# robflynnyh/dynamic-asr-eval

Measured on AMD Instinct MI355X. Metric: audio-sec/s dynamic-eval (fwd+1 adapt step), higher is better.
Workload: dtype f32; 1 GPU; run_dynamic_eval_full: 1 h Earnings-22-shape recording per step (360000 frames, seq_len 16384, overlap 14336, offline, MADGRAD lr 9e-05, 6 freq masks <=34), SCConformerXL 6x768 V+1=4096 seeded weights; windows_per_recording=169, chains_per_gpu=2, lockstep_group=4, hip_graphs=True, pcie_inclusive=False

## Files before the change

### dynamic-asr-eval_amd/csrc/ctc.hip

```cpp
#include "common.h"
#include "libm_f32.h"

namespace {

namespace glm = dyn::glm;

constexpr int SCAN_T = 1024;
template <int ITEMS> struct ScanCfg { static constexpr int PD = ITEMS >= 8 ? 2 : ITEMS >= 4 ? 4 : 8; };

__device__ __forceinline__ bool better(float v, int i, float bv, int bi) { return v > bv || (v == bv && i < bi); }

__global__ __launch_bounds__(256) void argmax_rows_kernel(const float* __restrict__ x, int32_t* __restrict__ ids,
                                                           int64_t rows, int C, int64_t ld, float* __restrict__ vals) {
    const int lane = threadIdx.x & 63, w = threadIdx.x >> 6;
    for (int64_t row = (int64_t)blockIdx.x * 4 + w; row < rows; row += (int64_t)gridDim.x * 4) {
        const float* xr = x + row * ld;
        float bv = -INFINITY;
        int bi = 0x7fffffff;
        for (int c = lane; c < C; c += 64) {
            const float v = xr[c];
            if (better(v, c, bv, bi)) { bv = v; bi = c; }
        }
#pragma unroll
        for (int o = 32; o > 0; o >>= 1) {
            const float ov = __shfl_xor(bv, o, 64);
            const int oi = __shfl_xor(bi, o, 64);
            if (better(ov, oi, bv, bi)) { bv = ov; bi = oi; }
        }
        if (lane == 0) {
            ids[row] = bi == 0x7fffffff ? 0 : bi;
            if (vals) vals[row] = bv;
        }
    }
}

__global__ __launch_bounds__(1024) void ctc_collapse_kernel(const int32_t* __restrict__ ids, int32_t* __restrict__ out,
                                                             int32_t* __restrict__ out_len, int64_t T, int64_t stride,
                                                             int blank) {
    __shared__ int wsum[16];
    __shared__ int base;
    const int64_t b = blockIdx.x;
    const int32_t* in = ids + b * stride;
    int32_t* o = out + b * stride;
    const int lane = threadIdx.x & 63, w = threadIdx.x >> 6;
    if (threadIdx.x == 0) base = 0;
    __syncthreads();
    for (int64_t t0 = 0; t0 < T; t0 += 1024) {
        const int64_t t = t0 + threadIdx.x;
        int id = -1, keep = 0;
        if (t < T) {
            id = in[t];
            const int prev = t > 0 ? in[t - 1] : -1;
            keep = (id != blank && id != prev) ? 1 : 0;
        }
        int incl = keep;
#pragma unroll
        for (int o2 = 1; o2 < 64; o2 <<= 1) {
            const int n = __shfl_up(incl, o2, 64);
            if (lane >= o2) incl += n;
        }
        if (lane == 63) wsum[w] = incl;
        __syncthreads();
        int woff = 0;
        for (int k = 0; k < w; ++k) woff += wsum[k];
        const int b0 = base;
        if (keep) o[b0 + woff + incl - 1] = id;
        __syncthreads();
        if (threadIdx.x == 1023) base = b0 + woff + incl;
        __syncthreads();
    }
    if (threadIdx.x == 0) out_len[b] = base;
}


struct CtcDims {
    int64_t T_max, B, C;
    int64_t lp_st, lp_sb;
    int64_t S_max;
    int64_t L_max;
    int blank;
};

__global__ __launch_bounds__(1024) void ctc_prep_kernel(const int32_t* __restrict__ targets, const int32_t* __restrict__ tlen,
                                                        int32_t* __restrict__ prev_same, int32_t* __restrict__ is_last,
                                                        int64_t S_max) {
    extern __shared__ int32_t tg_s[];
    const int64_t b = blockIdx.x;
    const int S = tlen[b];
    const int32_t* tg = targets + b * S_max;
    for (int k = threadIdx.x; k < S; k += blockDim.x) tg_s[k] = tg[k];
    __syncthreads();
    const int lane = threadIdx.x & 63, w = threadIdx.x >> 6, nw = blockDim.x >> 6;
    for (int k = w; k < S; k += nw) {
        const int c = tg_s[k];
        int pv = -1;
        for (int j0 = k - 1; j0 >= 0; j0 -= 64) {
            const int j = j0 - lane;
            const unsigned long long hit = __ballot(j >= 0 && tg_s[j] == c);
            if (hit) { pv = j0 - (__ffsll((long long)hit) - 1); break; }
        }
        int last = 1;
        for (int j0 = k + 1; j0 < S; j0 += 64) {
            const int j = j0 + lane;
            if (__ballot(j < S && tg_s[j] == c)) { last = 0; break; }
        }
        if (lane == 0) {
            prev_same[b * S_max + k] = pv;
            is_last[b * S_max + k] = last;
        }
    }
}

__global__ __launch_bounds__(256) void ctc_gather_kernel(const float* __restrict__ lp, const int32_t* __restrict__ targets,
                                                          const int32_t* __restrict__ ilen, const int32_t* __restrict__ tlen,
                                                          float* __restrict__ slab, CtcDims d) {
    const int64_t t = blockIdx.x, b = blockIdx.y;
    if (t >= ilen[b]) return;
    const int L = 2 * tlen[b] + 1;
    const float* row = lp + t * d.lp_st + b * d.lp_sb;
    const int32_t* tg = targets + b * d.S_max;
    float* out = slab + (b * d.T_max + t) * d.L_max;
    for (int s = threadIdx.x; s < L; s += blockDim.x) out[s] = row[(s & 1) ? tg[s >> 1] : d.blank];
}

__device__ __forceinline__ float lse3(float a, float b, float c, const double* tab) {
    float m = fmaxf(a, fmaxf(b, c));
    if (m == -INFINITY) m = 0.f;
    const float e = __fadd_rn(__fadd_rn(glm::exp_nonpos(__fsub_rn(a, m), tab), glm::exp_nonpos(__fsub_rn(b, m), tab)), glm::exp_nonpos(__fsub_rn(c, m), tab));
    return __fadd_rn(glm::logf_(e, tab), m);
}

template <int ITEMS>
__device__ __forceinline__ void ctc_alpha_body(float* rows, const double* tab, const float* __restrict__ slab, const int32_t* __restrict__ targets,
                                               const int32_t* __restrict__ ilen, const int32_t* __restrict__ tlen,
                                               float* __restrict__ alpha, float* __restrict__ nll, const CtcDims& d) {
    const int SCAN_T = blockDim.x;
    const int64_t b = blockIdx.x;
    const int T = ilen[b], S = tlen[b], L = 2 * S + 1;
    const int32_t* tg = targets + b * d.S_max;
    const float* sl = slab + b * d.T_max * d.L_max;
    float* al = alpha + b * d.T_max * d.L_max;
    float* prev = rows;
    float* cur = rows + d.L_max;
    constexpr int PD = ScanCfg<ITEMS>::PD;
    bool skip[ITEMS];
    float ring[ITEMS][PD];
#pragma unroll
    for (int j = 0; j < ITEMS; ++j) {
        const int s = threadIdx.x + j * SCAN_T;
        skip[j] = (s < L) && (s & 1) && s >= 3 && tg[s >> 1] != tg[(s >> 1) - 1];
        float v = -INFINITY;
        if (s < L && T > 0) {
            if (s == 0) v = sl[0];
            else if (s == 1) v = sl[1];
            al[s] = v;
            prev[s] = v;
        }
#pragma unroll
        for (int u = 0; u < PD; ++u) ring[j][u] = (s < L && 1 + u < T) ? sl[(int64_t)(1 + u) * d.L_max + s] : 0.f;
    }
    __syncthreads();
    for (int t0 = 1; t0 < T; t0 += PD) {
#pragma unroll
        for (int u = 0; u < PD; ++u) {
            const int t = t0 + u;
            if (t < T) {
#pragma unroll
                for (int j = 0; j < ITEMS; ++j) {
                    const int s = threadIdx.x + j * SCAN_T;
                    const float lpv = ring[j][u];
                    const int tn = t + PD;
                    ring[j][u] = (s < L && tn < T) ? sl[(int64_t)tn * d.L_max + s] : 0.f;
                    if (s < L) {
                        const float a = prev[s];
                        const float bb = s >= 1 ? prev[s - 1] : -INFINITY;
                        const float c = skip[j] ? prev[s - 2] : -INFINITY;
                        const float v = __fadd_rn(lse3(a, bb, c, tab), lpv);
                        cur[s] = v;
                        al[(int64_t)t * d.L_max + s] = v;
                    }
                }
                __syncthreads();
                float* tmp = prev; prev = cur; cur = tmp;
            }
        }
    }
    if (threadIdx.x == 0) {
        float r = INFINITY;
        if (T > 0) {
            const float l1 = prev[L - 1];
            if (S == 0) r = -l1;
            else {
                const float l2 = prev[L - 2];
                float m = fmaxf(l1, l2);
                if (m == -INFINITY) m = 0.f;
                r = -__fadd_rn(glm::logf_(__fadd_rn(glm::exp_nonpos(__fsub_rn(l1, m), tab), glm::exp_nonpos(__fsub_rn(l2, m), tab)), tab), m);
            }
        }
        nll[b] = r;
    }
}

template <int ITEMS>
__device__ __forceinline__ void ctc_beta_body(float* rows, const double* tab, const float* __restrict__ slab, const int32_t* __restrict__ targets,
                                              const int32_t* __restrict__ ilen, const int32_t* __restrict__ tlen,
                                              float* __restrict__ alpha, const CtcDims& d) {
    const int SCAN_T = blockDim.x;
    const int64_t b = blockIdx.x;
    const int T = ilen[b], S = tlen[b], L = 2 * S + 1;
    if (T <= 0) return;
    const int32_t* tg = targets + b * d.S_max;
    const float* sl = slab + b * d.T_max * d.L_max;
    float* al = alpha + b * d.T_max * d.L_max;
    float* prev = rows;
    float* cur = rows + d.L_max;
    constexpr int PD = ScanCfg<ITEMS>::PD;
    bool skip[ITEMS];
    float ring[ITEMS][PD];
#pragma unroll
    for (int j = 0; j < ITEMS; ++j) {
        const int s = threadIdx.x + j * SCAN_T;
        skip[j] = (s + 2 < L) && (s & 1) && tg[s >> 1] != tg[(s >> 1) + 1];
        if (s < L) {
            float v = -INFINITY;
            if (s == L - 1 || s == L - 2) v = sl[(int64_t)(T - 1) * d.L_max + s];
            prev[s] = v;
            al[(int64_t)(T - 1) * d.L_max + s] = v;
        }
#pragma unroll
        for (int u = 0; u < PD; ++u) {
            const int t = T - 2 - u;
            ring[j][u] = (s < L && t >= 0) ? sl[(int64_t)t * d.L_max + s] : 0.f;
        }
    }
    __syncthreads();
    for (int t0 = T - 2; t0 >= 0; t0 -= PD) {
#pragma unroll
        for (int u = 0; u < PD; ++u) {
            const int t = t0 - u;
            if (t >= 0) {
#pragma unroll
                for (int j = 0; j < ITEMS; ++j) {
                    const int s = threadIdx.x + j * SCAN_T;
                    const float lpv = ring[j][u];
                    const int tn = t - PD;
                    ring[j][u] = (s < L && tn >= 0) ? sl[(int64_t)tn * d.L_max + s] : 0.f;
                    if (s < L) {
                        const float a = prev[s];
                        const float bb = s + 1 < L ? prev[s + 1] : -INFINITY;
                        const float c = skip[j] ? prev[s + 2] : -INFINITY;
                        const float v = __fadd_rn(lse3(a, bb, c, tab), lpv);
                        cur[s] = v;
                        al[(int64_t)t * d.L_max + s] = v;
                    }
                }
                __syncthreads();
                float* tmp = prev; prev = cur; cur = tmp;
            }
        }
    }
}

template <int ITEMS>
__global__ __launch_bounds__(1024) void ctc_scan_kernel(const float* __restrict__ slab, const int32_t* __restrict__ targets,
                                                         const int32_t* __restrict__ ilen, const int32_t* __restrict__ tlen,
                                                         float* __restrict__ alpha, float* __restrict__ beta, float* __restrict__ nll,
                                                         CtcDims d) {
    extern __shared__ __attribute__((aligned(16))) double scan_lds[];
    glm::stage_table(scan_lds);
    float* rows = (float*)(scan_lds + glm::TABLE_DOUBLES);
    if (blockIdx.y == 0) ctc_alpha_body<ITEMS>(rows, scan_lds, slab, targets, ilen, tlen, alpha, nll, d);
    else ctc_beta_body<ITEMS>(rows, scan_lds, slab, targets, ilen, tlen, beta, d);
}

__device__ __forceinline__ float log_add_pair(float lcab, float ab, const double* tab) {
    if (lcab == -INFINITY) return ab;
    const float mx = lcab < ab ? ab : lcab;
    return __fadd_rn(glm::logf_(__fadd_rn(glm::exp_nonpos(__fsub_rn(lcab, mx), tab), glm::exp_nonpos(__fsub_rn(ab, mx), tab)), tab), mx);
}

__global__ __launch_bounds__(256) void ctc_grad_kernel(const float* __restrict__ lp, const float* __restrict__ alpha_,
                                                        const float* __restrict__ beta_,
                                                        const int32_t* __restrict__ targets, const int32_t* __restrict__ prev_same,
                                                        const int32_t* __restrict__ is_last, const int32_t* __restrict__ ilen, const int32_t* __restrict__ tlen,
                                                        const float* __restrict__ nll, float* __restrict__ grad, int64_t g_st,
                                                        int64_t g_sb, float grad_scale, int mean_reduction, CtcDims d) {
    extern __shared__ __attribute__((aligned(16))) double grad_lds[];
    const int64_t t = blockIdx.x, b = blockIdx.y;
    const int T = ilen[b], S = tlen[b], L = 2 * S + 1;
    float* gr = grad + t * g_st + b * g_sb;
    if (t >= T) {
        for (int c = threadIdx.x; c < d.C; c += blockDim.x) gr[c] = 0.f;
        return;
    }
    const double* tab = grad_lds;
    float* ab = (float*)(grad_lds + glm::TABLE_DOUBLES);
    glm::stage_table(grad_lds);
    float g = grad_scale;
    if (mean_reduction) g = (grad_scale / (float)d.B) / (float)(S > 0 ? S : 1);
    const float* row = lp + t * d.lp_st + b * d.lp_sb;
    const float* ar = alpha_ + (b * d.T_max + t) * d.L_max;
    const float* br = beta_ + (b * d.T_max + t) * d.L_max;
    const int32_t* tg = targets + b * d.S_max;
    const int32_t* pv = prev_same + b * d.S_max;
    const float nl = nll[b];
    for (int s = threadIdx.x; s < L; s += blockDim.x) ab[s] = __fadd_rn(ar[s], br[s]);
    __syncthreads();
    for (int c = threadIdx.x; c < d.C; c += blockDim.x) gr[c] = __fmul_rn(glm::expf_(row[c], tab), g);
    __syncthreads();
    if (threadIdx.x == 0) {
        float lcab = -INFINITY;
        for (int k = S; k >= 0; --k) lcab = log_add_pair(lcab, ab[2 * k], tab);
        const float lpb = row[d.blank];
        gr[d.blank] = __fmul_rn(__fsub_rn(glm::expf_(lpb, tab), glm::expf_(__fsub_rn(__fadd_rn(lcab, nl), lpb), tab)), g);
    }
    for (int k = (int)threadIdx.x - 64; k < S; k += (int)blockDim.x - 64) {
        if (k < 0 || !is_last[b * d.S_max + k]) continue;
        const int c = tg[k];
        float lcab = -INFINITY;
        for (int j = k; j >= 0; j = pv[j]) lcab = log_add_pair(lcab, ab[2 * j + 1], tab);
        const float lpc = row[c];
        gr[c] = __fmul_rn(__fsub_rn(glm::expf_(lpc, tab), glm::expf_(__fsub_rn(__fadd_rn(lcab, nl), lpc), tab)), g);
    }
}

__global__ void ctc_loss_reduce_kernel(const float* __restrict__ nll, const int32_t* __restrict__ tlen, float* loss, int64_t B,
                                       int mean_reduction) {
    if (threadIdx.x != 0 || blockIdx.x != 0) return;
    float s = 0.f;
    for (int64_t b = 0; b < B; ++b) {
        const int S = tlen[b];
        s += mean_reduction ? nll[b] / (float)(S > 0 ? S : 1) : nll[b];
    }
    *loss = mean_reduction ? s / (float)B : s;
}

inline int64_t align_up(int64_t v, int64_t a) { return (v + a - 1) / a * a; }

struct CtcWs {
    float* slab; float* alpha; float* beta; float* nll; int32_t* prev_same; int32_t* is_last;
    int64_t total;
};

CtcWs carve(void* ws, int64_t T, int64_t B, int64_t S_max) {
    const int64_t L = 2 * S_max + 1;
    CtcWs w;
    char* p = (char*)ws;
    int64_t off = 0;
    w.slab = (float*)(p + off); off += align_up(B * T * L * 4, 256);
    w.alpha = (float*)(p + off); off += align_up(B * T * L * 4, 256);
    w.beta = (float*)(p + off); off += align_up(B * T * L * 4, 256);
    w.nll = (float*)(p + off); off += align_up(B * 4, 256);
    w.prev_same = (int32_t*)(p + off); off += align_up((B * S_max + 1) * 4, 256);
    w.is_last = (int32_t*)(p + off); off += align_up((B * S_max + 1) * 4, 256);
    w.total = off;
    return w;
}

}

extern "C" int dyn_ctc_greedy(const float* log_probs, int64_t B, int64_t T, int64_t C, int64_t ld, int32_t blank,
                              int32_t* argmax_ids, int32_t* out_ids, int32_t* out_len, void* stream) {
    DYN_REQUIRE(log_probs && argmax_ids && out_ids && out_len && B >= 0 && T >= 0 && C > 0 && ld >= C, DYN_E_ARG,
                "dyn_ctc_greedy: bad arguments");
    if (B == 0) return DYN_OK;
    hipStream_t st = (hipStream_t)stream;
    if (T > 0) {
        int64_t g = dyn::cdiv(B * T, 4);
        if (g > 8192) g = 8192;
        hipLaunchKernelGGL(argmax_rows_kernel, dim3((unsigned)g), dim3(256), 0, st, log_probs, argmax_ids, B * T, (int)C, ld, (float*)nullptr);
    }
    hipLaunchKernelGGL(ctc_collapse_kernel, dim3((unsigned)B), dim3(1024), 0, st, argmax_ids, out_ids, out_len, T, T, (int)blank);
    return dyn::check_launch("dyn_ctc_greedy");
}

extern "C" int dyn_argmax_rows(const float* x, int64_t rows, int64_t C, int64_t ld, int32_t* ids, float* vals, void* stream) {
    DYN_REQUIRE(x && ids && rows >= 0 && C > 0 && ld >= C, DYN_E_ARG, "dyn_argmax_rows: bad arguments");
    if (rows == 0) return DYN_OK;
    int64_t g = dyn::cdiv(rows, 4);
    if (g > 8192) g = 8192;
    hipLaunchKernelGGL(argmax_rows_kernel, dim3((unsigned)g), dim3(256), 0, (hipStream_t)stream, x, ids, rows, (int)C, ld, vals);
    return dyn::check_launch("dyn_argmax_rows");
}

extern "C" int64_t dyn_ctc_loss_workspace_bytes(int64_t T, int64_t B, int64_t S_max) {
    return carve(nullptr, T, B, S_max > 0 ? S_max : 1).total;
}

extern "C" int dyn_ctc_loss_workspace_layout(int64_t T, int64_t B, int64_t S_max, int64_t* offsets4, int64_t* row_len) {
    DYN_REQUIRE(offsets4 && row_len && T > 0 && B > 0 && S_max >= 0, DYN_E_ARG, "dyn_ctc_loss_workspace_layout: bad arguments");
    const int64_t Sm = S_max > 0 ? S_max : 1;
    const CtcWs w = carve(nullptr, T, B, Sm);
    offsets4[0] = (char*)w.slab - (char*)nullptr;
    offsets4[1] = (char*)w.alpha - (char*)nullptr;
    offsets4[2] = (char*)w.beta - (char*)nullptr;
    offsets4[3] = (char*)w.nll - (char*)nullptr;
    *row_len = 2 * Sm + 1;
    return DYN_OK;
}

namespace {
__global__ __launch_bounds__(256) void libm_f32_kernel(const float* __restrict__ x, int64_t n, float* y_exp, float* y_log, float* y_np) {
    __shared__ double tab[glm::TABLE_DOUBLES];
    glm::stage_table(tab);
    __syncthreads();
    for (int64_t i = (int64_t)blockIdx.x * blockDim.x + threadIdx.x; i < n; i += (int64_t)gridDim.x * blockDim.x) {
        const float v = x[i];
        if (y_exp) y_exp[i] = glm::expf_(v, tab);
        if (y_log) y_log[i] = glm::logf_(v, tab);
        if (y_np) y_np[i] = glm::exp_nonpos(v, tab);
    }
}
}

extern "C" int dyn_libm_f32(const float* x, int64_t n, float* y_exp, float* y_log, float* y_exp_nonpos, void* stream) {
    DYN_REQUIRE(x && n >= 0, DYN_E_ARG, "dyn_libm_f32: bad arguments");
    if (n == 0) return DYN_OK;
    int64_t g = dyn::cdiv(n, 256);
    if (g > 4096) g = 4096;
    hipLaunchKernelGGL(libm_f32_kernel, dim3((unsigned)g), dim3(256), 0, (hipStream_t)stream, x, n, y_exp, y_log, y_exp_nonpos);
    return dyn::check_launch("dyn_libm_f32");
}

extern "C" int dyn_ctc_loss(const float* log_probs, int64_t T, int64_t B, int64_t C, int64_t lp_stride_t, int64_t lp_stride_b,
                            const int32_t* targets, int64_t S_max, const int32_t* input_lengths, const int32_t* target_lengths,
                            int32_t blank, int32_t reduction, float grad_scale, float* loss, float* nll_per_sample,
                            float* grad, int64_t g_stride_t, int64_t g_stride_b, void* workspace, int64_t workspace_bytes,
                            void* stream) {
    DYN_REQUIRE(log_probs && targets && input_lengths && target_lengths && loss && T > 0 && B > 0 && C > 0 && S_max >= 0 &&
                    blank >= 0 && blank < C && (reduction == 0 || reduction == 1),
                DYN_E_ARG, "dyn_ctc_loss: bad arguments");
    const int64_t Sm = S_max > 0 ? S_max : 1;
    const int64_t L = 2 * Sm + 1;
    DYN_REQUIRE(L <= 8 * SCAN_T, DYN_E_UNSUPPORTED, "dyn_ctc_loss: lattice width %lld > %d unsupported", (long long)L, 8 * SCAN_T);
    CtcWs w = carve(workspace, T, B, Sm);
    DYN_REQUIRE(workspace && workspace_bytes >= w.total, DYN_E_WORKSPACE, "dyn_ctc_loss: workspace %lld < %lld bytes",
                (long long)workspace_bytes, (long long)w.total);
    CtcDims d;
    d.T_max = T; d.B = B; d.C = C; d.lp_st = lp_stride_t; d.lp_sb = lp_stride_b; d.S_max = Sm; d.L_max = L; d.blank = blank;
    hipStream_t st = (hipStream_t)stream;
    hipLaunchKernelGGL(ctc_prep_kernel, dim3((unsigned)B), dim3(1024), (size_t)Sm * sizeof(int32_t), st, targets, target_lengths, w.prev_same, w.is_last, Sm);
    hipLaunchKernelGGL(ctc_gather_kernel, dim3((unsigned)T, (unsigned)B), dim3(256), 0, st, log_probs, targets, input_lengths,
                       target_lengths, w.slab, d);
    int threads = (int)((L + 63) / 64 * 64);
    if (threads > SCAN_T) threads = SCAN_T;
    const int items = (int)dyn::cdiv(L, threads);
    const size_t shm = (size_t)2 * L * sizeof(float) + glm::TABLE_DOUBLES * sizeof(double);
    const dim3 sgrid((unsigned)B, grad ? 2u : 1u);
#define GO_S(I) hipLaunchKernelGGL((ctc_scan_kernel<I>), sgrid, dim3(threads), shm, st, w.slab, targets, input_lengths, target_lengths, w.alpha, w.beta, w.nll, d)
    if (items <= 1) GO_S(1); else if (items <= 2) GO_S(2); else if (items <= 4) GO_S(4); else GO_S(8);
    hipLaunchKernelGGL(ctc_loss_reduce_kernel, dim3(1), dim3(64), 0, st, w.nll, target_lengths, loss, B, (int)reduction);
    if (nll_per_sample) {
        hipError_t e = hipMemcpyAsync(nll_per_sample, w.nll, B * sizeof(float), hipMemcpyDeviceToDevice, st);
        DYN_REQUIRE(e == hipSuccess, DYN_E_LAUNCH, "dyn_ctc_loss: copy of per-sample nll failed");
    }
    if (grad) {
        hipLaunchKernelGGL(ctc_grad_kernel, dim3((unsigned)T, (unsigned)B), dim3(256), (size_t)L * sizeof(float) + glm::TABLE_DOUBLES * sizeof(double), st, log_probs, w.alpha, w.beta, targets,
                           w.prev_same, w.is_last, input_lengths, target_lengths, w.nll, grad, g_stride_t, g_stride_b, grad_scale,
                           (int)reduction, d);
    }
#undef GO_S
    return dyn::check_launch("dyn_ctc_loss");
}
```

### dynamic-asr-eval_amd/csrc/libm_f32.h

```cpp
#pragma once
#include <stdint.h>

namespace dyn { namespace glm {

#if defined(__HIPCC__)
#define DYN_GLM_HD __host__ __device__ __forceinline__
#else
#define DYN_GLM_HD static inline
#endif

#define DYN_GLM_EXP_TABLE                                                                                              \
    0x3ff0000000000000ull, 0x3fefd9b0d3158574ull, 0x3fefb5586cf9890full, 0x3fef9301d0125b51ull, 0x3fef72b83c7d517bull, \
    0x3fef54873168b9aaull, 0x3fef387a6e756238ull, 0x3fef1e9df51fdee1ull, 0x3fef06fe0a31b715ull, 0x3feef1a7373aa9cbull, \
    0x3feedea64c123422ull, 0x3feece086061892dull, 0x3feebfdad5362a27ull, 0x3feeb42b569d4f82ull, 0x3feeab07dd485429ull, \
    0x3feea47eb03a5585ull, 0x3feea09e667f3bcdull, 0x3fee9f75e8ec5f74ull, 0x3feea11473eb0187ull, 0x3feea589994cce13ull, \
    0x3feeace5422aa0dbull, 0x3feeb737b0cdc5e5ull, 0x3feec49182a3f090ull, 0x3feed503b23e255dull, 0x3feee89f995ad3adull, \
    0x3feeff76f2fb5e47ull, 0x3fef199bdd85529cull, 0x3fef3720dcef9069ull, 0x3fef5818dcfba487ull, 0x3fef7c97337b9b5full, \
    0x3fefa4afa2a490daull, 0x3fefd0765b6e4540ull
#define DYN_GLM_LOG_TABLE                                                                                 \
    0x1.661ec79f8f3bep+0, -0x1.57bf7808caadep-2, 0x1.571ed4aaf883dp+0, -0x1.2bef0a7c06ddbp-2,               \
    0x1.49539f0f010b0p+0, -0x1.01eae7f513a67p-2, 0x1.3c995b0b80385p+0, -0x1.b31d8a68224e9p-3,               \
    0x1.30d190c8864a5p+0, -0x1.6574f0ac07758p-3, 0x1.25e227b0b8ea0p+0, -0x1.1aa2bc79c8100p-3,               \
    0x1.1bb4a4a1a343fp+0, -0x1.a4e76ce8c0e5ep-4, 0x1.12358f08ae5bap+0, -0x1.1973c5a611cccp-4,               \
    0x1.0953f419900a7p+0, -0x1.252f438e10c1ep-5, 0x1.0000000000000p+0, 0x0.0p+0,                            \
    0x1.e608cfd9a47acp-1, 0x1.aa5aa5df25984p-5, 0x1.ca4b31f026aa0p-1, 0x1.c5e53aa362eb4p-4,                 \
    0x1.b2036576afce6p-1, 0x1.526e57720db08p-3, 0x1.9c2d163a1aa2dp-1, 0x1.bc2860d224770p-3,                 \
    0x1.886e6037841edp-1, 0x1.1058bc8a07ee1p-2, 0x1.767dcf5534862p-1, 0x1.4043057b6ee09p-2

constexpr int TABLE_DOUBLES = 32 + 32;

#if defined(__HIP_DEVICE_COMPILE__)
DYN_GLM_HD double fma_(double a, double b, double c) { return __fma_rn(a, b, c); }
DYN_GLM_HD double mul_(double a, double b) { return __dmul_rn(a, b); }
DYN_GLM_HD double add_(double a, double b) { return __dadd_rn(a, b); }
DYN_GLM_HD uint64_t d2u(double d) { return (uint64_t)__double_as_longlong(d); }
DYN_GLM_HD double u2d(uint64_t u) { return __longlong_as_double((long long)u); }
DYN_GLM_HD uint32_t f2u(float f) { return __float_as_uint(f); }
DYN_GLM_HD float u2f(uint32_t u) { return __uint_as_float(u); }
#else
}}
#include <math.h>
#include <string.h>
namespace dyn { namespace glm {
DYN_GLM_HD double fma_(double a, double b, double c) { return fma(a, b, c); }
DYN_GLM_HD double mul_(double a, double b) { volatile double r = a * b; return r; }
DYN_GLM_HD double add_(double a, double b) { volatile double r = a + b; return r; }
DYN_GLM_HD uint64_t d2u(double d) { uint64_t u; memcpy(&u, &d, 8); return u; }
DYN_GLM_HD double u2d(uint64_t u) { double d; memcpy(&d, &u, 8); return d; }
DYN_GLM_HD uint32_t f2u(float f) { uint32_t u; memcpy(&u, &f, 4); return u; }
DYN_GLM_HD float u2f(uint32_t u) { float f; memcpy(&f, &u, 4); return f; }
#endif

DYN_GLM_HD float exp_core(float x, const double* tab) {
    const double xd = (double)x;
    const double InvLn2N = 0x1.71547652b82fep+5, SHIFT = 0x1.8p+52;
    const double C0 = 0x1.c6af84b912394p-20, C1 = 0x1.ebfce50fac4f3p-13, C2 = 0x1.62e42ff0c52d6p-6;
    const double z = mul_(InvLn2N, xd);
    double kd = add_(z, SHIFT);
    const uint64_t ki = d2u(kd);
    kd = add_(kd, -SHIFT);
    const double r = fma_(InvLn2N, xd, -kd);
    const uint64_t t = d2u(tab[ki & 31]) + (ki << 47);
    const double s = u2d(t);
    const double p = fma_(C0, r, C1);
    const double r2 = mul_(r, r);
    double y = fma_(C2, r, 1.0);
    y = fma_(p, r2, y);
    y = mul_(y, s);
    return (float)y;
}

DYN_GLM_HD float expf_(float x, const double* tab) {
    const uint32_t ux = f2u(x);
    const uint32_t abstop = (ux >> 20) & 0x7ff;
    if (abstop >= 0x42b) {
        if (ux == 0xff800000u) return 0.f;
        if (abstop >= 0x7f8) return x + x;
        if (x > 0x1.62e42ep6f) return u2f(0x7f800000u);
        if (x < -0x1.9fe368p6f) return 0.f;
    }
    return exp_core(x, tab);
}

DYN_GLM_HD float exp_nonpos(float x, const double* tab) {
    const float e = exp_core(x, tab);
    return x < -0x1.9fe368p6f ? 0.f : e;
}

DYN_GLM_HD float logf_(float x, const double* tab) {
    uint32_t ix = f2u(x);
    if (ix == 0x3f800000u) return 0.f;
    if (ix - 0x00800000u >= 0x7f800000u - 0x00800000u) {
        if (ix * 2 == 0) return u2f(0xff800000u);
        if (ix == 0x7f800000u) return x;
        if ((ix & 0x80000000u) || ix * 2 >= 0xff000000u) return u2f(0x7fc00000u);
        ix = f2u(x * 0x1p23f);
        ix -= 23u << 23;
    }
    const double A0 = -0x1.00ea348b88334p-2, A1 = 0x1.5575b0be00b6ap-2, A2 = -0x1.ffffef20a4123p-2, Ln2 = 0x1.62e42fefa39efp-1;
    const uint32_t tmp = ix - 0x3f330000u;
    const int i = (tmp >> 19) & 15;
    const int k = (int32_t)tmp >> 23;
    const uint32_t iz = ix - (tmp & 0xff800000u);
    const double invc = tab[32 + 2 * i], logc = tab[32 + 2 * i + 1];
    const double z = (double)u2f(iz);
    const double r = fma_(z, invc, -1.0);
    const double y0 = fma_((double)k, Ln2, logc);
    const double r2 = mul_(r, r);
    double y = fma_(A1, r, A2);
    y = fma_(A0, r2, y);
    y = fma_(y, r2, add_(y0, r));
    return (float)y;
}

#if defined(__HIPCC__)
static __device__ const uint64_t EXP_BITS_D[32] = {DYN_GLM_EXP_TABLE};
static __device__ const double LOG_PAIRS_D[32] = {DYN_GLM_LOG_TABLE};
__device__ __forceinline__ void stage_table(double* lds_tab) {
    for (int i = threadIdx.x; i < TABLE_DOUBLES; i += blockDim.x) lds_tab[i] = i < 32 ? u2d(EXP_BITS_D[i]) : LOG_PAIRS_D[i - 32];
}
#endif
static inline void fill_table_host(double* tab) {
    const uint64_t e[32] = {DYN_GLM_EXP_TABLE};
    const double l[32] = {DYN_GLM_LOG_TABLE};
    for (int i = 0; i < 32; ++i) {
        uint64_t u = e[i];
        double d;
        __builtin_memcpy(&d, &u, 8);
        tab[i] = d;
        tab[32 + i] = l[i];
    }
}

}}
```

Before: 794.7 audio-s/s.

## Restructure CTC scan by label parity with band skipping and parallel blank-gradient chains

The alpha/beta scan is merged into one templated routine where each wave handles only blank or only label positions. Blank lanes use a cheaper two-term log-sum-exp, and whole groups of states that are still unreachable early in time are skipped. Log-sum-exp now saves one exp by reusing the max term, and it calls a branch-free log that only handles inputs between 1 and 3. The serial blank-gradient chain, which ran on one thread per frame, moves to extra grid blocks that process 64 frames each with prefetched loads. The risks are more complex indexing and exactness that depends on the new lse formulations still matching bitwise.

Result: no change. 800.9 audio-s/s (median of 6 runs) (+0.8%).

```diff
diff --git a/dynamic-asr-eval_amd/csrc/ctc.hip b/dynamic-asr-eval_amd/csrc/ctc.hip
--- a/dynamic-asr-eval_amd/csrc/ctc.hip
+++ b/dynamic-asr-eval_amd/csrc/ctc.hip
@@ -1,9 +1,11 @@
 #include "common.h"
 #include "libm_f32.h"
+#include "ctc_lse.h"
 
 namespace {
 
 namespace glm = dyn::glm;
+namespace lse = dyn::lse;
 
 constexpr int SCAN_T = 1024;
 template <int ITEMS> struct ScanCfg { static constexpr int PD = ITEMS >= 8 ? 2 : ITEMS >= 4 ? 4 : 8; };
@@ -123,142 +125,78 @@
     for (int s = threadIdx.x; s < L; s += blockDim.x) out[s] = row[(s & 1) ? tg[s >> 1] : d.blank];
 }
 
-__device__ __forceinline__ float lse3(float a, float b, float c, const double* tab) {
-    float m = fmaxf(a, fmaxf(b, c));
-    if (m == -INFINITY) m = 0.f;
-    const float e = __fadd_rn(__fadd_rn(glm::exp_nonpos(__fsub_rn(a, m), tab), glm::exp_nonpos(__fsub_rn(b, m), tab)), glm::exp_nonpos(__fsub_rn(c, m), tab));
-    return __fadd_rn(glm::logf_(e, tab), m);
-}
-
-template <int ITEMS>
-__device__ __forceinline__ void ctc_alpha_body(float* rows, const double* tab, const float* __restrict__ slab, const int32_t* __restrict__ targets,
-                                               const int32_t* __restrict__ ilen, const int32_t* __restrict__ tlen,
-                                               float* __restrict__ alpha, float* __restrict__ nll, const CtcDims& d) {
-    const int SCAN_T = blockDim.x;
-    const int64_t b = blockIdx.x;
-    const int T = ilen[b], S = tlen[b], L = 2 * S + 1;
-    const int32_t* tg = targets + b * d.S_max;
-    const float* sl = slab + b * d.T_max * d.L_max;
-    float* al = alpha + b * d.T_max * d.L_max;
+__device__ __forceinline__ void lds_barrier() {
+    __builtin_amdgcn_fence(__ATOMIC_RELEASE, "workgroup", "local");
+    __builtin_amdgcn_s_barrier();
+    __builtin_amdgcn_fence(__ATOMIC_ACQUIRE, "workgroup", "local");
+}
+
+template <int ITEMS, bool BETA, int PAR>
+__device__ __forceinline__ void ctc_scan_steps(float* rows, const double* tab, const float* __restrict__ sl, const int32_t* __restrict__ tg,
+                                               float* __restrict__ lat, int T, int S, int64_t Lm, int64_t rstep) {
+    constexpr int PD = ScanCfg<ITEMS>::PD;
+    constexpr int NB1 = BETA ? 1 : -1;
+    const int L = 2 * S + 1;
+    const int w = __builtin_amdgcn_readfirstlane((int)threadIdx.x >> 6), lane = threadIdx.x & 63;
+    const int kitem = ((int)blockDim.x >> 7) * 64;
     float* prev = rows;
-    float* cur = rows + d.L_max;
-    constexpr int PD = ScanCfg<ITEMS>::PD;
-    bool skip[ITEMS];
+    float* cur = rows + Lm;
+    int s[ITEMS], sc[ITEMS], band[ITEMS];
+    bool live[ITEMS], skip[ITEMS];
     float ring[ITEMS][PD];
 #pragma unroll
     for (int j = 0; j < ITEMS; ++j) {
-        const int s = threadIdx.x + j * SCAN_T;
-        skip[j] = (s < L) && (s & 1) && s >= 3 && tg[s >> 1] != tg[(s >> 1) - 1];
+        const int k0 = (w >> 1) * 64 + j * kitem, k = k0 + lane;
+        s[j] = 2 * k + PAR;
+        live[j] = s[j] < L;
+        sc[j] = live[j] ? s[j] : 0;
+        skip[j] = false;
+        if (PAR && live[j]) skip[j] = BETA ? (k + 1 < S && tg[k] != tg[k + 1]) : (k >= 1 && tg[k] != tg[k - 1]);
+        const int smin = 2 * k0 + PAR, smax = min(smin + 126, L - 1);
+        band[j] = BETA ? L - 1 - smax : smin;
         float v = -INFINITY;
-        if (s < L && T > 0) {
-            if (s == 0) v = sl[0];
-            else if (s == 1) v = sl[1];
-            al[s] = v;
-            prev[s] = v;
-        }
-#pragma unroll
-        for (int u = 0; u < PD; ++u) ring[j][u] = (s < L && 1 + u < T) ? sl[(int64_t)(1 + u) * d.L_max + s] : 0.f;
-    }
-    __syncthreads();
-    for (int t0 = 1; t0 < T; t0 += PD) {
-#pragma unroll
-        for (int u = 0; u < PD; ++u) {
-            const int t = t0 + u;
-            if (t < T) {
-#pragma unroll
-                for (int j = 0; j < ITEMS; ++j) {
-                    const int s = threadIdx.x + j * SCAN_T;
-                    const float lpv = ring[j][u];
-                    const int tn = t + PD;
-                    ring[j][u] = (s < L && tn < T) ? sl[(int64_t)tn * d.L_max + s] : 0.f;
-                    if (s < L) {
-                        const float a = prev[s];
-                        const float bb = s >= 1 ? prev[s - 1] : -INFINITY;
-                        const float c = skip[j] ? prev[s - 2] : -INFINITY;
-                        const float v = __fadd_rn(lse3(a, bb, c, tab), lpv);
-                        cur[s] = v;
-                        al[(int64_t)t * d.L_max + s] = v;
-                    }
+        if (live[j]) {
+            if (BETA ? s[j] >= L - 2 : s[j] <= 1) v = sl[s[j]];
+            lat[s[j]] = v;
+            prev[s[j]] = v;
+        }
+#pragma unroll
+        for (int u = 0; u < PD; ++u) ring[j][u] = sl[(int64_t)min(1 + u, T - 1) * rstep + sc[j]];
+    }
+    lds_barrier();
+    auto step = [&](int n, int u, bool prefetch) {
+#pragma unroll
+        for (int j = 0; j < ITEMS; ++j) {
+            const float lpv = ring[j][u];
+            if (band[j] > 2 * n + 1) {
+                if (live[j]) {
+                    cur[s[j]] = -INFINITY;
+                    lat[(int64_t)n * rstep + s[j]] = -INFINITY;
                 }
-                __syncthreads();
-                float* tmp = prev; prev = cur; cur = tmp;
+            } else if (live[j]) {
+                const int nb = s[j] + NB1;
+                const float a = prev[s[j]];
+                const float bb = (PAR || (BETA ? nb < L : nb >= 0)) ? prev[nb] : -INFINITY;
+                float x;
+                if (PAR) x = lse::lse3(a, bb, skip[j] ? prev[s[j] + 2 * NB1] : -INFINITY, tab);
+                else x = lse::lse2(a, bb, tab);
+                const float v = __fadd_rn(x, lpv);
+                cur[s[j]] = v;
+                lat[(int64_t)n * rstep + s[j]] = v;
             }
-        }
-    }
-    if (threadIdx.x == 0) {
-        float r = INFINITY;
-        if (T > 0) {
-            const float l1 = prev[L - 1];
-            if (S == 0) r = -l1;
-            else {
-                const float l2 = prev[L - 2];
-                float m = fmaxf(l1, l2);
-                if (m == -INFINITY) m = 0.f;
-                r = -__fadd_rn(glm::logf_(__fadd_rn(glm::exp_nonpos(__fsub_rn(l1, m), tab), glm::exp_nonpos(__fsub_rn(l2, m), tab)), tab), m);
-            }
-        }
-        nll[b] = r;
-    }
-}
-
-template <int ITEMS>
-__device__ __forceinline__ void ctc_beta_body(float* rows, const double* tab, const float* __restrict__ slab, const int32_t* __restrict__ targets,
-                                              const int32_t* __restrict__ ilen, const int32_t* __restrict__ tlen,
-                                              float* __restrict__ alpha, const CtcDims& d) {
-    const int SCAN_T = blockDim.x;
-    const int64_t b = blockIdx.x;
-    const int T = ilen[b], S = tlen[b], L = 2 * S + 1;
-    if (T <= 0) return;
-    const int32_t* tg = targets + b * d.S_max;
-    const float* sl = slab + b * d.T_max * d.L_max;
-    float* al = alpha + b * d.T_max * d.L_max;
-    float* prev = rows;
-    float* cur = rows + d.L_max;
-    constexpr int PD = ScanCfg<ITEMS>::PD;
-    bool skip[ITEMS];
-    float ring[ITEMS][PD];
-#pragma unroll
-    for (int j = 0; j < ITEMS; ++j) {
-        const int s = threadIdx.x + j * SCAN_T;
-        skip[j] = (s + 2 < L) && (s & 1) && tg[s >> 1] != tg[(s >> 1) + 1];
-        if (s < L) {
-            float v = -INFINITY;
-            if (s == L - 1 || s == L - 2) v = sl[(int64_t)(T - 1) * d.L_max + s];
-            prev[s] = v;
-            al[(int64_t)(T - 1) * d.L_max + s] = v;
-        }
-#pragma unroll
-        for (int u = 0; u < PD; ++u) {
-            const int t = T - 2 - u;
-            ring[j][u] = (s < L && t >= 0) ? sl[(int64_t)t * d.L_max + s] : 0.f;
-        }
-    }
-    __syncthreads();
-    for (int t0 = T - 2; t0 >= 0; t0 -= PD) {
-#pragma unroll
-        for (int u = 0; u < PD; ++u) {
-            const int t = t0 - u;
-            if (t >= 0) {
-#pragma unroll
-                for (int j = 0; j < ITEMS; ++j) {
-                    const int s = threadIdx.x + j * SCAN_T;
-                    const float lpv = ring[j][u];
-                    const int tn = t - PD;
-                    ring[j][u] = (s < L && tn >= 0) ? sl[(int64_t)tn * d.L_max + s] : 0.f;
-                    if (s < L) {
-                        const float a = prev[s];
-                        const float bb = s + 1 < L ? prev[s + 1] : -INFINITY;
-                        const float c = skip[j] ? prev[s + 2] : -INFINITY;
-                        const float v = __fadd_rn(lse3(a, bb, c, tab), lpv);
-                        cur[s] = v;
-                        al[(int64_t)t * d.L_max + s] = v;
-                    }
-                }
-                __syncthreads();
-                float* tmp = prev; prev = cur; cur = tmp;
-            }
-        }
-    }
+            if (prefetch) ring[j][u] = sl[(int64_t)min(n + PD, T - 1) * rstep + sc[j]];
+        }
+        lds_barrier();
+        float* tmp = prev; prev = cur; cur = tmp;
+    };
+    int n0 = 1;
+    for (; n0 + PD <= T; n0 += PD) {
+#pragma unroll
+        for (int u = 0; u < PD; ++u) step(n0 + u, u, true);
+    }
+#pragma unroll
+    for (int u = 0; u < PD - 1; ++u)
+        if (n0 + u < T) step(n0 + u, u, false);
 }
 
 template <int ITEMS>
@@ -269,31 +207,96 @@
     extern __shared__ __attribute__((aligned(16))) double scan_lds[];
     glm::stage_table(scan_lds);
     float* rows = (float*)(scan_lds + glm::TABLE_DOUBLES);
-    if (blockIdx.y == 0) ctc_alpha_body<ITEMS>(rows, scan_lds, slab, targets, ilen, tlen, alpha, nll, d);
-    else ctc_beta_body<ITEMS>(rows, scan_lds, slab, targets, ilen, tlen, beta, d);
-}
-
-__device__ __forceinline__ float log_add_pair(float lcab, float ab, const double* tab) {
-    if (lcab == -INFINITY) return ab;
-    const float mx = lcab < ab ? ab : lcab;
-    return __fadd_rn(glm::logf_(__fadd_rn(glm::exp_nonpos(__fsub_rn(lcab, mx), tab), glm::exp_nonpos(__fsub_rn(ab, mx), tab)), tab), mx);
-}
+    const int64_t b = blockIdx.x;
+    const bool backward = blockIdx.y != 0;
+    const int T = ilen[b], S = tlen[b], L = 2 * S + 1;
+    if (T <= 0) {
+        if (!backward && threadIdx.x == 0) nll[b] = INFINITY;
+        return;
+    }
+    const int32_t* tg = targets + b * d.S_max;
+    const int64_t base = b * d.T_max * d.L_max;
+    const int w = threadIdx.x >> 6;
+    const bool label_wave = ((w >> 2) + w) & 1;
+    if (backward) {
+        const int64_t last = base + (int64_t)(T - 1) * d.L_max;
+        if (label_wave) ctc_scan_steps<ITEMS, true, 1>(rows, scan_lds, slab + last, tg, beta + last, T, S, d.L_max, -d.L_max);
+        else ctc_scan_steps<ITEMS, true, 0>(rows, scan_lds, slab + last, tg, beta + last, T, S, d.L_max, -d.L_max);
+        return;
+    }
+    if (label_wave) ctc_scan_steps<ITEMS, false, 1>(rows, scan_lds, slab + base, tg, alpha + base, T, S, d.L_max, d.L_max);
+    else ctc_scan_steps<ITEMS, false, 0>(rows, scan_lds, slab + base, tg, alpha + base, T, S, d.L_max, d.L_max);
+    if (threadIdx.x == 0) {
+        const float* fin = rows + ((T - 1) & 1 ? d.L_max : 0);
+        const float l1 = fin[L - 1];
+        nll[b] = S == 0 ? -l1 : -lse::lse2(l1, fin[L - 2], scan_lds);
+    }
+}
+
+constexpr int GRAD_TL = 64;
+constexpr int GRAD_PD = 8;
 
 __global__ __launch_bounds__(256) void ctc_grad_kernel(const float* __restrict__ lp, const float* __restrict__ alpha_,
                                                         const float* __restrict__ beta_,
                                                         const int32_t* __restrict__ targets, const int32_t* __restrict__ prev_same,
                                                         const int32_t* __restrict__ is_last, const int32_t* __restrict__ ilen, const int32_t* __restrict__ tlen,
                                                         const float* __restrict__ nll, float* __restrict__ grad, int64_t g_st,
-                                                        int64_t g_sb, float grad_scale, int mean_reduction, CtcDims d) {
+                                                        int64_t g_sb, float grad_scale, int mean_reduction, int64_t chain_blocks, CtcDims d) {
     extern __shared__ __attribute__((aligned(16))) double grad_lds[];
-    const int64_t t = blockIdx.x, b = blockIdx.y;
-    const int T = ilen[b], S = tlen[b], L = 2 * S + 1;
+    const double* tab = grad_lds;
+    const int64_t nchain = d.B * chain_blocks;
+    if ((int64_t)blockIdx.x < nchain) {
+        const int64_t b = blockIdx.x / chain_blocks, t0 = (blockIdx.x % chain_blocks) * GRAD_TL;
+        const int T = ilen[b], S = tlen[b];
+        if (t0 >= T) return;
+        glm::stage_table(grad_lds);
+        __syncthreads();
+        if (threadIdx.x >= GRAD_TL) return;
+        const int64_t t = t0 + threadIdx.x;
+        const bool act = t < T;
+        const int64_t row_off = (b * d.T_max + (act ? t : T - 1)) * d.L_max;
+        const float* ar = alpha_ + row_off;
+        const float* br = beta_ + row_off;
+        float ra[GRAD_PD], rb[GRAD_PD];
+#pragma unroll
+        for (int u = 0; u < GRAD_PD; ++u) {
+            const int k = S - u;
+            ra[u] = ar[2 * max(k, 0)];
+            rb[u] = br[2 * max(k, 0)];
+        }
+        float lcab = -INFINITY;
+        auto link = [&](int k, int u, bool prefetch) {
+            lcab = lse::log_add_pair(lcab, __fadd_rn(ra[u], rb[u]), tab);
+            if (prefetch) {
+                ra[u] = ar[2 * max(k - GRAD_PD, 0)];
+                rb[u] = br[2 * max(k - GRAD_PD, 0)];
+            }
+        };
+        int k0 = S;
+        for (; k0 - (GRAD_PD - 1) >= 0; k0 -= GRAD_PD) {
+#pragma unroll
+            for (int u = 0; u < GRAD_PD; ++u) link(k0 - u, u, true);
+        }
+#pragma unroll
+        for (int u = 0; u < GRAD_PD - 1; ++u)
+            if (k0 - u >= 0) link(k0 - u, u, false);
+        if (act) {
+            float g = grad_scale;
+            if (mean_reduction) g = (grad_scale / (float)d.B) / (float)(S > 0 ? S : 1);
+            const float lpb = lp[t * d.lp_st + b * d.lp_sb + d.blank];
+            grad[t * g_st + b * g_sb + d.blank] =
+                __fmul_rn(__fsub_rn(glm::expf_(lpb, tab), glm::expf_(__fsub_rn(__fadd_rn(lcab, nll[b]), lpb), tab)), g);
+        }
+        return;
+    }
+    const int64_t row_id = (int64_t)blockIdx.x - nchain;
+    const int64_t b = row_id / d.T_max, t = row_id % d.T_max;
+    const int T = ilen[b], S = tlen[b];
     float* gr = grad + t * g_st + b * g_sb;
     if (t >= T) {
         for (int c = threadIdx.x; c < d.C; c += blockDim.x) gr[c] = 0.f;
         return;
     }
-    const double* tab = grad_lds;
     float* ab = (float*)(grad_lds + glm::TABLE_DOUBLES);
     glm::stage_table(grad_lds);
     float g = grad_scale;
@@ -304,21 +307,16 @@
     const int32_t* tg = targets + b * d.S_max;
     const int32_t* pv = prev_same + b * d.S_max;
     const float nl = nll[b];
-    for (int s = threadIdx.x; s < L; s += blockDim.x) ab[s] = __fadd_rn(ar[s], br[s]);
+    for (int k = threadIdx.x; k < S; k += blockDim.x) ab[k] = __fadd_rn(ar[2 * k + 1], br[2 * k + 1]);
     __syncthreads();
-    for (int c = threadIdx.x; c < d.C; c += blockDim.x) gr[c] = __fmul_rn(glm::expf_(row[c], tab), g);
+    for (int c = threadIdx.x; c < d.C; c += blockDim.x)
+        if (c != d.blank) gr[c] = __fmul_rn(glm::expf_(row[c], tab), g);
     __syncthreads();
-    if (threadIdx.x == 0) {
-        float lcab = -INFINITY;
-        for (int k = S; k >= 0; --k) lcab = log_add_pair(lcab, ab[2 * k], tab);
-        const float lpb = row[d.blank];
-        gr[d.blank] = __fmul_rn(__fsub_rn(glm::expf_(lpb, tab), glm::expf_(__fsub_rn(__fadd_rn(lcab, nl), lpb), tab)), g);
-    }
-    for (int k = (int)threadIdx.x - 64; k < S; k += (int)blockDim.x - 64) {
-        if (k < 0 || !is_last[b * d.S_max + k]) continue;
+    for (int k = threadIdx.x; k < S; k += blockDim.x) {
+        if (!is_last[b * d.S_max + k]) continue;
         const int c = tg[k];
         float lcab = -INFINITY;
-        for (int j = k; j >= 0; j = pv[j]) lcab = log_add_pair(lcab, ab[2 * j + 1], tab);
+        for (int j = k; j >= 0; j = pv[j]) lcab = lse::log_add_pair(lcab, ab[j], tab);
         const float lpc = row[c];
         gr[c] = __fmul_rn(__fsub_rn(glm::expf_(lpc, tab), glm::expf_(__fsub_rn(__fadd_rn(lcab, nl), lpc), tab)), g);
     }
@@ -442,9 +440,10 @@
     hipLaunchKernelGGL(ctc_prep_kernel, dim3((unsigned)B), dim3(1024), (size_t)Sm * sizeof(int32_t), st, targets, target_lengths, w.prev_same, w.is_last, Sm);
     hipLaunchKernelGGL(ctc_gather_kernel, dim3((unsigned)T, (unsigned)B), dim3(256), 0, st, log_probs, targets, input_lengths,
                        target_lengths, w.slab, d);
-    int threads = (int)((L + 63) / 64 * 64);
-    if (threads > SCAN_T) threads = SCAN_T;
-    const int items = (int)dyn::cdiv(L, threads);
+    int pair_waves = (int)dyn::cdiv(Sm + 1, 64);
+    if (pair_waves > SCAN_T / 128) pair_waves = SCAN_T / 128;
+    const int threads = 128 * pair_waves;
+    const int items = (int)dyn::cdiv(Sm + 1, 64 * pair_waves);
     const size_t shm = (size_t)2 * L * sizeof(float) + glm::TABLE_DOUBLES * sizeof(double);
     const dim3 sgrid((unsigned)B, grad ? 2u : 1u);
 #define GO_S(I) hipLaunchKernelGGL((ctc_scan_kernel<I>), sgrid, dim3(threads), shm, st, w.slab, targets, input_lengths, target_lengths, w.alpha, w.beta, w.nll, d)
@@ -455,9 +454,11 @@
         DYN_REQUIRE(e == hipSuccess, DYN_E_LAUNCH, "dyn_ctc_loss: copy of per-sample nll failed");
     }
     if (grad) {
-        hipLaunchKernelGGL(ctc_grad_kernel, dim3((unsigned)T, (unsigned)B), dim3(256), (size_t)L * sizeof(float) + glm::TABLE_DOUBLES * sizeof(double), st, log_probs, w.alpha, w.beta, targets,
+        const int64_t chain_blocks = dyn::cdiv(T, GRAD_TL);
+        DYN_REQUIRE(B * (chain_blocks + T) <= 0x7fffffffLL, DYN_E_UNSUPPORTED, "dyn_ctc_loss: %lld x %lld frames exceed one gradient grid", (long long)B, (long long)T);
+        hipLaunchKernelGGL(ctc_grad_kernel, dim3((unsigned)(B * (chain_blocks + T))), dim3(256), (size_t)Sm * sizeof(float) + glm::TABLE_DOUBLES * sizeof(double), st, log_probs, w.alpha, w.beta, targets,
                            w.prev_same, w.is_last, input_lengths, target_lengths, w.nll, grad, g_stride_t, g_stride_b, grad_scale,
-                           (int)reduction, d);
+                           (int)reduction, chain_blocks, d);
     }
 #undef GO_S
     return dyn::check_launch("dyn_ctc_loss");
diff --git a/dynamic-asr-eval_amd/csrc/ctc_lse.h b/dynamic-asr-eval_amd/csrc/ctc_lse.h
--- /dev/null
+++ b/dynamic-asr-eval_amd/csrc/ctc_lse.h
@@ -0,0 +1,49 @@
+#pragma once
+#include "libm_f32.h"
+
+namespace dyn { namespace lse {
+
+namespace glm = dyn::glm;
+
+#if defined(__HIP_DEVICE_COMPILE__)
+DYN_GLM_HD float addf(float a, float b) { return __fadd_rn(a, b); }
+DYN_GLM_HD float subf(float a, float b) { return __fsub_rn(a, b); }
+#else
+DYN_GLM_HD float addf(float a, float b) { volatile float r = a + b; return r; }
+DYN_GLM_HD float subf(float a, float b) { volatile float r = a - b; return r; }
+#endif
+
+DYN_GLM_HD float lse2(float a, float b, const double* tab) {
+    float m = fmaxf(a, b);
+    if (m == -INFINITY) m = 0.f;
+    const float da = subf(a, m), db = subf(b, m);
+    const bool amax = da == 0.f, bmax = db == 0.f;
+    const float ex = glm::exp_nonpos(amax ? db : da, tab);
+    const float ea = amax ? 1.f : ex;
+    const float eb = amax ? ex : bmax ? 1.f : ex;
+    return addf(glm::log_1to3(addf(ea, eb), tab), m);
+}
+
+DYN_GLM_HD float lse3(float a, float b, float c, const double* tab) {
+    float m = fmaxf(a, fmaxf(b, c));
+    if (m == -INFINITY) m = 0.f;
+    const float da = subf(a, m), db = subf(b, m), dc = subf(c, m);
+    const bool amax = da == 0.f, bmax = !amax && db == 0.f, cmax = !amax && !bmax && dc == 0.f;
+    const float ex = glm::exp_nonpos(amax ? db : da, tab);
+    const float ey = glm::exp_nonpos(cmax ? db : dc, tab);
+    const float ea = amax ? 1.f : ex;
+    const float eb = bmax ? 1.f : amax ? ex : ey;
+    const float ec = cmax ? 1.f : ey;
+    return addf(glm::log_1to3(addf(addf(ea, eb), ec), tab), m);
+}
+
+DYN_GLM_HD float log_add_pair(float lcab, float ab, const double* tab) {
+    const float mx = lcab < ab ? ab : lcab;
+    const float d1 = subf(lcab, mx), d2 = subf(ab, mx);
+    const bool first = d1 == 0.f;
+    const float ex = glm::exp_nonpos(first ? d2 : d1, tab);
+    const float r = addf(glm::log_1to3(addf(first ? 1.f : ex, first ? ex : 1.f), tab), mx);
+    return lcab == -INFINITY ? ab : r;
+}
+
+}}
diff --git a/dynamic-asr-eval_amd/csrc/libm_f32.h b/dynamic-asr-eval_amd/csrc/libm_f32.h
--- a/dynamic-asr-eval_amd/csrc/libm_f32.h
+++ b/dynamic-asr-eval_amd/csrc/libm_f32.h
@@ -87,16 +87,7 @@
     return x < -0x1.9fe368p6f ? 0.f : e;
 }
 
-DYN_GLM_HD float logf_(float x, const double* tab) {
-    uint32_t ix = f2u(x);
-    if (ix == 0x3f800000u) return 0.f;
-    if (ix - 0x00800000u >= 0x7f800000u - 0x00800000u) {
-        if (ix * 2 == 0) return u2f(0xff800000u);
-        if (ix == 0x7f800000u) return x;
-        if ((ix & 0x80000000u) || ix * 2 >= 0xff000000u) return u2f(0x7fc00000u);
-        ix = f2u(x * 0x1p23f);
-        ix -= 23u << 23;
-    }
+DYN_GLM_HD float log_core(uint32_t ix, const double* tab) {
     const double A0 = -0x1.00ea348b88334p-2, A1 = 0x1.5575b0be00b6ap-2, A2 = -0x1.ffffef20a4123p-2, Ln2 = 0x1.62e42fefa39efp-1;
     const uint32_t tmp = ix - 0x3f330000u;
     const int i = (tmp >> 19) & 15;
@@ -111,6 +102,24 @@
     y = fma_(A0, r2, y);
     y = fma_(y, r2, add_(y0, r));
     return (float)y;
+}
+
+DYN_GLM_HD float logf_(float x, const double* tab) {
+    uint32_t ix = f2u(x);
+    if (ix == 0x3f800000u) return 0.f;
+    if (ix - 0x00800000u >= 0x7f800000u - 0x00800000u) {
+        if (ix * 2 == 0) return u2f(0xff800000u);
+        if (ix == 0x7f800000u) return x;
+        if ((ix & 0x80000000u) || ix * 2 >= 0xff000000u) return u2f(0x7fc00000u);
+        ix = f2u(x * 0x1p23f);
+        ix -= 23u << 23;
+    }
+    return log_core(ix, tab);
+}
+
+DYN_GLM_HD float log_1to3(float x, const double* tab) {
+    const float y = log_core(f2u(x), tab);
+    return x == 0.f ? u2f(0xff800000u) : y;
 }
 
 #if defined(__HIPCC__)
```
